# anulum/scpn-fusion-core

Measured on NVIDIA B200. Metric: converged_equilibria_per_s, higher is better.
Workload: dtype f64

## Files before the change

### scpn_fusion_core_b200/csrc/gsb_picard.cu

```cuda
#include "gsb_internal.cuh"
#include "gsb_resident.cuh"

#include <algorithm>
#include <cstdlib>

constexpr int kPT = 32;
constexpr int kTW = 8;
constexpr int kRW = 4;
constexpr int kSadChunk = 4096;
constexpr int kSadChunksMax = 64;

struct PicardState {
  int *active, *status, *iter, *cur, *best, *nxt, *xsel, *seed_active;
  double *diff_best, *gs_best, *gs_last, *diff_last, *scale;
  double *axbnd;
  double *topo;
};

struct Bufs {
  double *p[3];
};

struct gsb_picard_ws {
  int cap = 0;
// ... 890 lines not shown
  s.cur[b] = 0;
  s.best[b] = best0;
  s.nxt[b] = 1;
  s.xsel[b] = -1;
  s.seed_active[b] = (on && seed && fabs(ip[b]) >= 1e-12) ? 1 : 0;
  s.diff_best[b] = 1e9;
  s.gs_best[b] = INFINITY;
  s.gs_last[b] = INFINITY;
  s.diff_last[b] = 0.0;
  s.scale[b] = 0.0;
}

__global__ void __launch_bounds__(256)
k_seed_source(size_t n, int nr, const double *__restrict__ seedJ, double seed_sum_drdz,
              const double *__restrict__ ip, const double *__restrict__ mr,
              double *__restrict__ jphi, double *__restrict__ source,
              const int *__restrict__ seed_active) {
  const int b = blockIdx.y;
  if (!seed_active[b]) return;
  const double sc = seed_sum_drdz > 0.0 ? __ddiv_rn(ip[b], seed_sum_drdz) : 1.0;
  for (size_t i = (size_t)blockIdx.x * blockDim.x + threadIdx.x; i < n; i += (size_t)gridDim.x * blockDim.x) {
    const double j = dmul(seedJ[i], sc);
    jphi[(size_t)b * n + i] = j;
    source[(size_t)b * n + i] = dmul(mr[i % nr], j);
  }
}

__global__ void __launch_bounds__(256)
k_finalize(Bufs bufs, PicardState s, size_t n, double *__restrict__ summary, int batch,
           const int *__restrict__ mask) {
  const int b = blockIdx.y;
  if (mask && !mask[b]) return;
  const int c = s.cur[b];
  if (c != 0) {
    const double *f = bufs.p[c] + (size_t)b * n;
    double *d = bufs.p[0] + (size_t)b * n;
    for (size_t i = (size_t)blockIdx.x * blockDim.x + threadIdx.x; i < n; i += (size_t)gridDim.x * blockDim.x)
      d[i] = f[i];
  }
  if (blockIdx.x == 0 && threadIdx.x == 0 && summary) {
    double *o = summary + (size_t)b * 16;
    const double *t = s.topo + (size_t)b * 8;
    o[0] = (double)s.iter[b];
    o[1] = s.status[b] == 1 ? 1.0 : 0.0;
    o[2] = s.diff_best[b];
    o[3] = s.gs_last[b];
    o[4] = s.gs_best[b];
    o[5] = (double)s.status[b];
    o[6] = s.axbnd[2 * b];
    o[7] = s.axbnd[2 * b + 1];
    o[8] = t[0];
    o[9] = t[1];
    o[10] = t[3];
    o[11] = t[4];
    o[12] = s.diff_last[b];
    o[13] = t[6];
    o[14] = s.scale[b];
    o[15] = 0.0;
  }
}

__global__ void __launch_bounds__(256)
k_bfield(const double *__restrict__ psi, int nz, int nr, GradGeom gg, const double *__restrict__ rrow,
         double *__restrict__ br, double *__restrict__ bz) {
  const int b = blockIdx.z;
  const int ir = blockIdx.x * blockDim.x + threadIdx.x;
  const int iz = blockIdx.y * blockDim.y + threadIdx.y;
  if (ir >= nr || iz >= nz) return;
  const size_t n = (size_t)nz * nr;
  double gz, gr;
  grad_point(psi + b * n, nz, nr, iz, ir, gg, gz, gr);
  const double rs = fmax(rrow[ir], 1e-6);
  const double inv = __ddiv_rn(1.0, rs);
  br[b * n + (size_t)iz * nr + ir] = dmul(-inv, gz);
  bz[b * n + (size_t)iz * nr + ir] = dmul(inv, gr);
}


struct PicardResArgs {
  double *psi;
  const double *bc;
  const double *ip;
  const double *prof_dev;
  double *jphi;
  double *summary;
  double *hist, *gs_hist;
  double *ws_psi;
  double *ws_src;
  const double *seedJ, *cf, *mr, *rrow;
  const int *rowmask;
  double seed_sum_drdz;
  int batch, max_iter, seed, saddle, need_gs, external;
  double tol, gs_tol, alpha, oma, omega;
  double dr, dz, dr2, dz2, four_drdz;
  GradGeom gg;
  ProfileDev prof;
  int scratch_off;
  int tplane_off;
  const int *order;
  const int *n_order;
};

__device__ __forceinline__ double pl(int xo, int nz, int hw, int iz, int ir) {
  return res_pool[xo + split_index(nz, hw, iz, ir)];
}

__device__ __forceinline__ void grad_planes(int xo, int nz, int nr, int hw, int iz, int ir, const GradGeom &gg,
                                            double &gz, double &gr) {
  const double c = pl(xo, nz, hw, iz, ir);
  if (iz == 0)
    gz = ddiv_y(dsub(pl(xo, nz, hw, 1, ir), c), gg.dz, gg.inv_dz);
  else if (iz == nz - 1)
    gz = ddiv_y(dsub(c, pl(xo, nz, hw, iz - 1, ir)), gg.dz, gg.inv_dz);
  else
    gz = ddiv_y(dsub(pl(xo, nz, hw, iz + 1, ir), pl(xo, nz, hw, iz - 1, ir)), gg.two_dz, gg.inv_two_dz);
  if (ir == 0)
    gr = ddiv_y(dsub(pl(xo, nz, hw, iz, 1), c), gg.dr, gg.inv_dr);
  else if (ir == nr - 1)
    gr = ddiv_y(dsub(c, pl(xo, nz, hw, iz, ir - 1)), gg.dr, gg.inv_dr);
  else
    gr = ddiv_y(dsub(pl(xo, nz, hw, iz, ir + 1), pl(xo, nz, hw, iz, ir - 1)), gg.two_dr, gg.inv_two_dr);
}

__device__ __forceinline__ double grad_mag(const GradGeom &gg, double c, double up, double down, double left,
                                           double right, bool z_lo, bool z_hi, bool r_lo, bool r_hi) {
  double gz, gr;
  if (z_lo)
    gz = ddiv_yf(dsub(up, c), gg.dz, gg.inv_dz);
  else if (z_hi)
    gz = ddiv_yf(dsub(c, down), gg.dz, gg.inv_dz);
  else
    gz = ddiv_yf(dsub(up, down), gg.two_dz, gg.inv_two_dz);
  if (r_lo)
    gr = ddiv_yf(dsub(right, c), gg.dr, gg.inv_dr);
  else if (r_hi)
    gr = ddiv_yf(dsub(c, left), gg.dr, gg.inv_dr);
  else
    gr = ddiv_yf(dsub(right, left), gg.two_dr, gg.inv_two_dr);
  return hypot_glibc(gr, gz);
}

struct JrawK {
  double psi_ax, denom, inv_denom;
  bool hmode, same_prof;
  MtanhK mkp, mkf;
};
__device__ __forceinline__ double jraw_point(const JrawK &K, double v, double r, double cfv) {
  const double pn = ddiv_yf(dsub(v, K.psi_ax), K.denom, K.inv_denom);
  double pr = 0.0, ff = 0.0;
  if (pn >= 0.0 && pn < 1.0) {
    if (K.hmode) {
      pr = mtanh_res(pn, K.mkp);
      ff = K.same_prof ? pr : mtanh_res(pn, K.mkf);
    } else {
      pr = ff = dsub(1.0, pn);
    }
  }
  return dadd(dmul(0.5, dmul(r, pr)), dmul(0.5, dmul(cfv, ff)));
}

__device__ __forceinline__ double bcast_d(double v, int slot_off) {
  __syncthreads();
  if (threadIdx.x == 0) res_pool[slot_off] = v;
  __syncthreads();
  return res_pool[slot_off];
}

__global__ void __launch_bounds__(kResThreads, 1)
k_picard_resident(const __grid_constant__ RPlan plan, const __grid_constant__ PicardResArgs a) {
  const int lev_off = res_stage(plan);
  int nz, nr, hw, xo, f_lk, f_nch, f_rpc, f_nk;
  ResK rk;
  {
    const RLevel &F = res_level(lev_off, 0);
    nz = F.nz, nr = F.nr, hw = F.hw, xo = F.x_off, f_lk = F.lk, f_nch = F.nch, f_rpc = F.rpc, f_nk = F.nk;
    rk = res_load_resk(F.g);
  }
  const double *tab_ae = plan.lev[0].g.a_e;
  const double *tab_rs = plan.lev[0].g.r_safe, *tab_irs = plan.lev[0].g.inv_r_safe;
  const double a_ns0 = plan.lev[0].g.a_ns, a_c0 = plan.lev[0].g.a_c, inv_a_c0 = plan.lev[0].g.inv_a_c;
  const int n = nz * nr, ps = nz * hw, planes = 2 * ps, nslot = ps;
  const int tid = threadIdx.x, T = blockDim.x;
  const int lane = tid & 31, warp = tid >> 5, nw = T >> 5;
  const int step_z = T / hw, step_k = T - step_z * hw;
  const int iz_first = tid / hw, k_first = tid - iz_first * hw;
  double *sh = res_pool + a.scratch_off;
  int *shi = reinterpret_cast<int *>(sh + 32);
  const int bslot = a.scratch_off + 48;
  double *wpsi = a.ws_psi + (size_t)blockIdx.x * 3 * planes;
  double *wsrc = a.ws_src + (size_t)blockIdx.x * planes;
  const double n_all = (double)n, n_int = (double)(nz - 2) * (double)(nr - 2);
  const bool odd_nr = (nr & 1) != 0;

#define GSB_SLOT_LOOP_BEGIN()                                                  \
  for (int e = tid, iz = iz_first, k = k_first; e < nslot; e += T) {          \
    const int par_ = iz & 1;                                                   \
    const int pa = par_ * ps + e, pb = (1 - par_) * ps + e;                    \
    const bool has_odd = odd_nr ? (k < hw - 1) : true;
#define GSB_SLOT_LOOP_END()                                                    \
    k += step_k;                                                               \
    iz += step_z;                                                              \
    if (k >= hw) {                                                             \
      k -= hw;                                                                 \
      ++iz;                                                                    \
    }                                                                          \
  }

  const int n_work = a.order ? min(*a.n_order, a.batch) : a.batch;
  for (int wi = blockIdx.x; wi < n_work; wi += gridDim.x) {
    const int b = a.order ? a.order[wi] : wi;
    const double *bc = a.bc + (size_t)b * n;
    const double ipb = a.ip[b];
    double pp[4], pf[4];
#pragma unroll
    for (int i = 0; i < 4; ++i) {
      pp[i] = a.prof_dev ? a.prof_dev[(size_t)b * 8 + i] : a.prof.p[i];
      pf[i] = a.prof_dev ? a.prof_dev[(size_t)b * 8 + 4 + i] : a.prof.f[i];
    }
    const MtanhK mkp = mtanh_k(pp), mkf = mtanh_k(pf);
    const bool same_prof = pp[0] == pf[0] && pp[1] == pf[1] && pp[2] == pf[2] && pp[3] == pf[3];
    __syncthreads();
    res_load_dense(a.psi + (size_t)b * n, xo, nz, nr, hw);
    int cur = 0, best = 0, nxt = 1;
    const bool do_seed = a.seed && fabs(ipb) >= 1e-12;
    const double seed_sc = a.seed_sum_drdz > 0.0 ? __ddiv_rn(ipb, a.seed_sum_drdz) : 1.0;
    __syncthreads();
    if (a.seed) {
      for (int i = tid; i < planes; i += T) wpsi[2 * planes + i] = res_pool[xo + i];
      best = 2;
    }

    if (do_seed) {
      const double sc = seed_sc;
      for (int iz = warp; iz < nz; iz += nw)
        for (int ir = lane; ir < nr; ir += 32) {
          const double j = dmul(a.seedJ[iz * nr + ir], sc);
          wsrc[split_index(nz, hw, iz, ir)] = dmul(a.mr[ir], j);
        }
      __syncthreads();
      int p0 = xo, p1 = xo + ps, pt = a.tplane_off;
      for (int step = 0; step < 50; ++step) {
#pragma unroll 1
        for (int c = 0; c < 2; ++c) {
          const int src_plane = c == 0 ? p0 : p1;
          const int oth_plane = c == 0 ? p1 : p0;
          const int dst_plane = c == 0 ? pt : p1;
          int o = tid, iz = iz_first, k = k_first;
          while (o < nslot) {
            int vo[4], vz[4], vk[4];
            double vf[4];
#pragma unroll
            for (int u = 0; u < 4; ++u) {
              vo[u] = o, vz[u] = iz, vk[u] = k;
              const int s = (c + iz) & 1;
              const int ir = 2 * k + s;
              const bool interior = o < nslot && ir < nr && iz > 0 && iz < nz - 1 && ir > 0 && ir < nr - 1;
              vf[u] = interior ? __ldcg(wsrc + c * ps + o) : 0.0;
              o += T, k += step_k, iz += step_z;
              if (k >= hw) k -= hw, ++iz;
            }
#pragma unroll
            for (int u = 0; u < 4; ++u) {
              const int oo = vo[u], zz = vz[u];
              const int s = (c + zz) & 1;
              const int ir = 2 * vk[u] + s;
              if (oo < nslot && ir < nr) {
                double v;
                if (zz == 0 || zz == nz - 1 || ir == 0 || ir == nr - 1) {
                  v = sanitize_fast(res_pool[src_plane + oo]);
                } else {
                  const double cc = sanitize_fast(res_pool[oth_plane + oo]);
                  const double side = sanitize_fast(res_pool[oth_plane + oo - 1 + 2 * s]);
                  const double S = sanitize_fast(res_pool[oth_plane + oo - hw]), N = sanitize_fast(res_pool[oth_plane + oo + hw]);
                  const double f = sanitize_fast(vf[u]);
                  double acc = dadd(dmul(__ldg(tab_ae + ir), s ? side : cc), dmul(__ldg(tab_ae + nr + ir), s ? cc : side));
                  acc = dadd(acc, dmul(a_ns0, S));
                  acc = dadd(acc, dmul(a_ns0, N));
                  acc = dsub(acc, f);
                  v = clip_cap(ddiv_y(acc, a_c0, inv_a_c0));
                }
                res_pool[dst_plane + oo] = v;
              }
            }
          }
          __syncthreads();
        }
        const int t = p0;
        p0 = pt;
        pt = t;
      }
    }
    if (a.external && !do_seed) {
      for (int i = tid; i < planes; i += T) wsrc[i] = 0.0;
    }
    __syncthreads();
    for (int i = tid; i < planes; i += T) wpsi[(size_t)cur * planes + i] = res_pool[xo + i];
    __syncthreads();

    int status = 0, iters = 0;
    int j_slot = -1;
    bool j_ok = false;
    double diff_best = 1e9, gs_best = INFINITY, gs_last = INFINITY, diff_last = 0.0, scale = 0.0;
    double psi_ax = 0.0, psi_b = 0.0, t_izax = 0, t_irax = 0, t_izx = 0, t_irx = 0, t_found = 0;

    for (int kit = 0; kit < a.max_iter; ++kit) {
      GSB_PHASE_BEGIN();
      ValIdx mx{0.0, -1}, mb{0.0, -1};
      double mn = INFINITY;
      GSB_SLOT_LOOP_BEGIN()
        const int flat = iz * nr + 2 * k;
        const double ve = res_pool[xo + pa];
        const double vo = has_odd ? res_pool[xo + pb] : ve;
        if (ve > mx.v || mx.i < 0) mx = ValIdx{ve, flat};
        mn = fmin(mn, ve);
        if (has_odd) {
          if (vo > mx.v) mx = ValIdx{vo, flat + 1};
          mn = fmin(mn, vo);
        }
        if (__ldg(a.rowmask + iz) != 0) {
          const bool z_lo = iz == 0, z_hi = iz == nz - 1;
          {
            const double up = z_hi ? 0.0 : res_pool[xo + pb + hw], down = z_lo ? 0.0 : res_pool[xo + pb - hw];
            const double left = k > 0 ? res_pool[xo + pb - 1] : 0.0;
            const double bm = grad_mag(a.gg, ve, up, down, left, vo, z_lo, z_hi, k == 0, !has_odd);
            if (isfinite(bm)) mb = better<false>(mb, ValIdx{bm, flat});
          }
          if (has_odd) {
            const bool r_hi = 2 * k + 1 == nr - 1;
            const double up = z_hi ? 0.0 : res_pool[xo + pa + hw], down = z_lo ? 0.0 : res_pool[xo + pa - hw];
            const double right = r_hi ? 0.0 : res_pool[xo + pa + 1];
            const double bm = grad_mag(a.gg, vo, up, down, ve, right, z_lo, z_hi, false, r_hi);
            if (isfinite(bm)) mb = better<false>(mb, ValIdx{bm, flat + 1});
          }
        }
      GSB_SLOT_LOOP_END()
      mx = block_arg<true>(mx, sh, shi);
      __syncthreads();
      mb = block_arg<false>(mb, sh, shi);
      __syncthreads();
      mn = -block_max(-mn, sh);
      int xi = mb.i;
      if (a.saddle) {
        double prev_v = -1.0, best_v = INFINITY;
        int prev_i = -1, best_i = -1;
        for (int round = 0; round < 16; ++round) {
          ValIdx c{0.0, -1};
          for (int iz = warp; iz < nz; iz += nw) {
            if (!a.rowmask[iz]) continue;
            for (int ir = lane; ir < nr; ir += 32) {
              const int flat = iz * nr + ir;
              double gz, gr;
              grad_planes(xo, nz, nr, hw, iz, ir, a.gg, gz, gr);
              const double bm = hypot_glibc(gr, gz);
              if (!isfinite(bm)) continue;
              if (bm < prev_v || (bm == prev_v && flat <= prev_i)) continue;
              c = better<false>(c, ValIdx{bm, flat});
            }
          }
          __syncthreads();
          c = block_arg<false>(c, sh, shi);
          if (threadIdx.x == 0) {
            res_pool[bslot] = c.v;
            res_pool[bslot + 1] = (double)c.i;
          }
          __syncthreads();
          prev_v = res_pool[bslot];
          prev_i = (int)res_pool[bslot + 1];
          __syncthreads();
          if (prev_i < 0) break;
          const int iz = prev_i / nr, ir = prev_i - iz * nr;
          if (iz > 0 && iz < nz - 1 && ir > 0 && ir < nr - 1) {
            const double q0 = pl(xo, nz, hw, iz, ir), c2 = dmul(2.0, q0);
            const double d2r = __ddiv_rn(dadd(dsub(pl(xo, nz, hw, iz, ir + 1), c2), pl(xo, nz, hw, iz, ir - 1)), a.dr2);
            const double d2z = __ddiv_rn(dadd(dsub(pl(xo, nz, hw, iz + 1, ir), c2), pl(xo, nz, hw, iz - 1, ir)), a.dz2);
            const double drz = __ddiv_rn(dadd(dsub(dsub(pl(xo, nz, hw, iz + 1, ir + 1), pl(xo, nz, hw, iz + 1, ir - 1)),
                                                   pl(xo, nz, hw, iz - 1, ir + 1)),
                                              pl(xo, nz, hw, iz - 1, ir - 1)),
                                         a.four_drdz);
            const double det = dsub(dmul(d2r, d2z), dmul(drz, drz));
            if (isfinite(det) && det < 0.0 && prev_v < best_v) {
              best_v = prev_v;
              best_i = prev_i;
            }
          }
        }
        if (best_i >= 0) xi = best_i;
      }
      if (threadIdx.x == 0) {
        double pax = mx.v;
        if (fabs(pax) < 1e-6) pax = 1e-6;
        double px;
        double fx = 0.0, izx = 0.0, irx = 0.0;
        if (xi >= 0) {
          const int iz = xi / nr, ir = xi - iz * nr;
          px = pl(xo, nz, hw, iz, ir);
          fx = 1.0;
          izx = iz;
          irx = ir;
        } else {
          px = mn;
        }
        double pb = px;
        if (fabs(dsub(pax, pb)) < 0.1) pb = dmul(pax, 0.1);
        res_pool[bslot] = pax;
        res_pool[bslot + 1] = pb;
        res_pool[bslot + 2] = (double)(mx.i / nr);
        res_pool[bslot + 3] = (double)(mx.i % nr);
        res_pool[bslot + 4] = izx;
        res_pool[bslot + 5] = irx;
        res_pool[bslot + 6] = fx;
      }
      __syncthreads();
      psi_ax = res_pool[bslot];
      psi_b = res_pool[bslot + 1];
      t_izax = res_pool[bslot + 2];
      t_irax = res_pool[bslot + 3];
      t_izx = res_pool[bslot + 4];
      t_irx = res_pool[bslot + 5];
      t_found = res_pool[bslot + 6];
      __syncthreads();
      GSB_PHASE(48);

      if (!a.external) {
      double denom = dsub(psi_b, psi_ax);
      if (fabs(denom) < 1e-9) denom = 1e-9;
      const double inv_denom = __ddiv_rn(1.0, denom);
      const bool hmode = a.prof.hmode != 0;
      j_slot = cur;
      double acc = 0.0;
      GSB_SLOT_LOOP_BEGIN()
        const double pn_e = ddiv_yf(dsub(res_pool[xo + pa], psi_ax), denom, inv_denom);
        const double pn_o = has_odd ? ddiv_yf(dsub(res_pool[xo + pb], psi_ax), denom, inv_denom) : -1.0;
        const bool in_e = pn_e >= 0.0 && pn_e < 1.0, in_o = pn_o >= 0.0 && pn_o < 1.0;
        double pr_e = 0.0, ff_e = 0.0, pr_o = 0.0, ff_o = 0.0;
        if (in_e || in_o) {
          if (hmode) {
            const double te = mtanh_res(pn_e, mkp), to = mtanh_res(pn_o, mkp);
            double fe = te, fo = to;
            if (!same_prof) {
              fe = mtanh_res(pn_e, mkf);
              fo = mtanh_res(pn_o, mkf);
            }
            pr_e = in_e ? te : 0.0, ff_e = in_e ? fe : 0.0;
            pr_o = in_o ? to : 0.0, ff_o = in_o ? fo : 0.0;
          } else {
            pr_e = ff_e = in_e ? dsub(1.0, pn_e) : 0.0;
            pr_o = ff_o = in_o ? dsub(1.0, pn_o) : 0.0;
          }
        }
        const double je = dadd(dmul(0.5, dmul(__ldg(a.rrow + 2 * k), pr_e)), dmul(0.5, dmul(__ldg(a.cf + 2 * k), ff_e)));
        __stcg(wsrc + pa, je);
        acc += je;
        if (has_odd) {
          const double jo = dadd(dmul(0.5, dmul(__ldg(a.rrow + 2 * k + 1), pr_o)), dmul(0.5, dmul(__ldg(a.cf + 2 * k + 1), ff_o)));
          __stcg(wsrc + pb, jo);
          acc += jo;
        }
      GSB_SLOT_LOOP_END()
      acc = block_sum(acc, sh);
      const double jsum = bcast_d(acc, bslot + 8);
      const double icur = dmul(dmul(jsum, a.dr), a.dz);
      const bool ok = fabs(icur) > 1e-9;
      scale = ok ? __ddiv_rn(ipb, icur) : 0.0;
      j_ok = ok;
      {
        int e = tid, iz = iz_first, k = k_first;
        while (e < nslot) {
          double vje[4], vjo[4];
          int vpa[4], vpb[4], vk[4];
          bool vok[4], vho[4];
#pragma unroll
          for (int u = 0; u < 4; ++u) {
            const int par_ = iz & 1;
            vok[u] = e < nslot;
            vpa[u] = par_ * ps + e, vpb[u] = (1 - par_) * ps + e, vk[u] = k;
            vho[u] = odd_nr ? (k < hw - 1) : true;
            vje[u] = vok[u] ? __ldcg(wsrc + vpa[u]) : 0.0;
            vjo[u] = (vok[u] && vho[u]) ? __ldcg(wsrc + vpb[u]) : 0.0;
            e += T, k += step_k, iz += step_z;
            if (k >= hw) k -= hw, ++iz;
          }
#pragma unroll
          for (int u = 0; u < 4; ++u) {
            if (vok[u]) {
              const double je = ok ? dmul(vje[u], scale) : 0.0;
              __stcg(wsrc + vpa[u], dmul(__ldg(a.mr + 2 * vk[u]), je));
              if (vho[u]) {
                const double jo = ok ? dmul(vjo[u], scale) : 0.0;
                __stcg(wsrc + vpb[u], dmul(__ldg(a.mr + 2 * vk[u] + 1), jo));
              }
            }
          }
        }
      }
      }
      __syncthreads();
      GSB_PHASE(49);

      res_vcycle(lev_off, plan.nlev, wsrc, a.omega, 3, 3);
      __syncthreads();
      GSB_PHASE(50);

      const double *old = wpsi + (size_t)cur * planes;
      double *out = wpsi + (size_t)nxt * planes;
      double dsum = 0.0;
      int bad = 0;
      {
        int e = tid, iz = iz_first, k = k_first;
        while (e < nslot) {
          double voe[4], voo[4];
          int vpa[4], vpb[4], vk[4], vz[4];
          bool vok[4], vho[4];
#pragma unroll
          for (int u = 0; u < 4; ++u) {
            const int par_ = iz & 1;
            vok[u] = e < nslot;
            vpa[u] = par_ * ps + e, vpb[u] = (1 - par_) * ps + e, vk[u] = k, vz[u] = iz;
            vho[u] = odd_nr ? (k < hw - 1) : true;
            voe[u] = vok[u] ? __ldcg(old + vpa[u]) : 0.0;
            voo[u] = (vok[u] && vho[u]) ? __ldcg(old + vpb[u]) : 0.0;
            e += T, k += step_k, iz += step_z;
            if (k >= hw) k -= hw, ++iz;
          }
#pragma unroll
          for (int u = 0; u < 4; ++u) {
            if (vok[u]) {
              const bool zwall = vz[u] == 0 || vz[u] == nz - 1;
              {
                const bool wall = zwall || vk[u] == 0 || !vho[u];
                const double wn = wall ? bc[vz[u] * nr + 2 * vk[u]] : res_pool[xo + vpa[u]];
                const double ov = voe[u];
                if (!(fabs(wn) <= 1.79769313486231570815e308)) bad = 1;
                dsum += fabs(dsub(wn, ov));
                const double c = dadd(dmul(a.oma, ov), dmul(a.alpha, wn));
                res_pool[xo + vpa[u]] = c;
                __stcg(out + vpa[u], c);
              }
              if (vho[u]) {
                const bool wall = zwall || (2 * vk[u] + 1 == nr - 1);
                const double wn = wall ? bc[vz[u] * nr + 2 * vk[u] + 1] : res_pool[xo + vpb[u]];
                const double ov = voo[u];
                if (!(fabs(wn) <= 1.79769313486231570815e308)) bad = 1;
                dsum += fabs(dsub(wn, ov));
                const double c = dadd(dmul(a.oma, ov), dmul(a.alpha, wn));
                res_pool[xo + vpb[u]] = c;
                __stcg(out + vpb[u], c);
              }
            }
          }
        }
      }
      const int anybad = __syncthreads_or(bad);
      GSB_PHASE(51);
      double rmax = 0.0, rsq = 0.0;
      {
        const int k = tid & ((1 << f_lk) - 1), ch = tid >> f_lk;
        const int z0 = 1 + ch * f_rpc;
        const int z1 = min(z0 + f_rpc, nz - 1);
        if (ch < f_nch && k < f_nk && z0 < z1) {
          const int ce = 2 * k, co = 2 * k + 1;
          const bool e_in = ce >= 1 && ce <= nr - 2, o_in = co <= nr - 2;
          const double rs_e = __ldg(tab_rs + ce), irs_e = __ldg(tab_irs + ce);
          const double rs_o = o_in ? __ldg(tab_rs + co) : 1.0, irs_o = o_in ? __ldg(tab_irs + co) : 1.0;
          int e = z0 * hw + k;
          int par = z0 & 1;
          double ev_m = res_pool[xo + (1 - par) * ps + e - hw], od_m = res_pool[xo + par * ps + e - hw];
          double ev_0 = res_pool[xo + par * ps + e], od_0 = res_pool[xo + (1 - par) * ps + e];
          for (int iz = z0; iz < z1; ++iz) {
            const int pa = par * ps + e, pb = (1 - par) * ps + e;
            const double ev_p = res_pool[xo + pb + hw], od_p = res_pool[xo + pa + hw];
            if (e_in) {
              const double w = res_pool[xo + pb - 1];
              const double r = dsub(res_lx(rk, rs_e, irs_e, ev_0, od_0, w, ev_m, ev_p), __ldcg(wsrc + pa));
              rmax = fmax(rmax, fabs(r));
              rsq += r * r;
            }
            if (o_in) {
              const double ee = res_pool[xo + pa + 1];
              const double r = dsub(res_lx(rk, rs_o, irs_o, od_0, ee, ev_0, od_m, od_p), __ldcg(wsrc + pb));
              rmax = fmax(rmax, fabs(r));
              rsq += r * r;
            }
            ev_m = ev_0, ev_0 = ev_p;
            od_m = od_0, od_0 = od_p;
            e += hw;
            par ^= 1;
          }
        }
      }
      dsum = block_sum(dsum, sh);
      __syncthreads();
      rmax = block_max(rmax, sh);
      __syncthreads();
      rsq = block_sum(rsq, sh);
      if (threadIdx.x == 0) {
        double code = 0.0;
        double dbest = diff_best, gbest = gs_best, dl = diff_last, gl = gs_last;
        double improved = 0.0;
        if (anybad) {
          code = 3.0;
        } else {
          const double diff = dsum / n_all;
          const double gs = (rmax > 0.0 && n_int > 0.0) ? sqrt(rsq / n_int) : 0.0;
          if (a.hist) a.hist[(size_t)b * a.max_iter + kit] = diff;
          if (a.gs_hist) a.gs_hist[(size_t)b * a.max_iter + kit] = gs;
          dl = diff;
          gl = gs;
          if (gs < gbest) gbest = gs;
          if (diff < dbest) {
            dbest = diff;
            improved = 1.0;
          }
          if (diff < a.tol && (!a.need_gs || gs < a.gs_tol))
            code = 1.0;
          else if (kit + 1 >= a.max_iter)
            code = 2.0;
        }
        res_pool[bslot] = code;
        res_pool[bslot + 1] = dbest;
        res_pool[bslot + 2] = gbest;
        res_pool[bslot + 3] = dl;
        res_pool[bslot + 4] = gl;
        res_pool[bslot + 5] = improved;
      }
      __syncthreads();
      const int code = (int)res_pool[bslot];
      diff_best = res_pool[bslot + 1];
      gs_best = res_pool[bslot + 2];
      diff_last = res_pool[bslot + 3];
      gs_last = res_pool[bslot + 4];
      const bool improved = res_pool[bslot + 5] != 0.0;
      __syncthreads();
      iters = kit + 1;
      GSB_PHASE(52);
      if (blockIdx.x == 0 && threadIdx.x == 0) GSB_PHASE_COUNT(53);
      if (code == 3) {
        status = 3;
        cur = best;
        break;
      }
      const int newcur = nxt;
      if (improved) best = newcur;
      cur = newcur;
      nxt = (cur == best) ? (cur == 0 ? 1 : 0) : 3 - cur - best;
      if (code != 0) {
        status = code;
        break;
      }
    }

    {
      const double *fin = wpsi + (size_t)cur * planes;
      const double *jsrc = wpsi + (size_t)(j_slot >= 0 ? j_slot : 0) * planes;
      JrawK jk;
      jk.psi_ax = psi_ax;
      jk.denom = dsub(psi_b, psi_ax);
      if (fabs(jk.denom) < 1e-9) jk.denom = 1e-9;
      jk.inv_denom = __ddiv_rn(1.0, jk.denom);
      jk.hmode = a.prof.hmode != 0, jk.same_prof = same_prof, jk.mkp = mkp, jk.mkf = mkf;
      double *po = a.psi + (size_t)b * n;
      double *jo = a.jphi + (size_t)b * n;
      for (int iz = warp; iz < nz; iz += nw)
        for (int ir = lane; ir < nr; ir += 32) {
          const int o = split_index(nz, hw, iz, ir);
          po[iz * nr + ir] = fin[o];
          double j;
          if (j_slot >= 0)
            j = j_ok ? dmul(jraw_point(jk, __ldcg(jsrc + o), __ldg(a.rrow + ir), __ldg(a.cf + ir)), scale) : 0.0;
          else
            j = do_seed ? dmul(a.seedJ[iz * nr + ir], seed_sc) : 0.0;
          jo[iz * nr + ir] = j;
        }
      if (threadIdx.x == 0 && a.summary) {
        double *o = a.summary + (size_t)b * 16;
        o[0] = (double)iters;
        o[1] = status == 1 ? 1.0 : 0.0;
        o[2] = diff_best;
        o[3] = gs_last;
        o[4] = gs_best;
        o[5] = (double)status;
        o[6] = psi_ax;
        o[7] = psi_b;
        o[8] = t_izax;
        o[9] = t_irax;
        o[10] = t_izx;
        o[11] = t_irx;
        o[12] = diff_last;
        o[13] = t_found;
        o[14] = scale;
        o[15] = 0.0;
      }
    }
    __syncthreads();
  }
#undef GSB_SLOT_LOOP_BEGIN
#undef GSB_SLOT_LOOP_END
}

__global__ void k_fb_init(int *__restrict__ mask, int *__restrict__ order, int *__restrict__ n_order,
                          double *__restrict__ fbsum, int batch) {
  const int b = blockIdx.x * blockDim.x + threadIdx.x;
  if (b == 0) *n_order = batch;
  if (b >= batch) return;
  mask[b] = 1;
  order[b] = b;
  fbsum[4 * b] = 0.0;
  fbsum[4 * b + 1] = INFINITY;
  fbsum[4 * b + 2] = 0.0;
  fbsum[4 * b + 3] = 0.0;
}

__device__ __forceinline__ int wall_index(int nz, int nr, int iz, int ir) {
  if (iz == 0) return ir;
  if (iz == nz - 1) return nr + 2 * (nz - 2) + ir;
  return nr + 2 * (iz - 1) + (ir ? 1 : 0);
}

__global__ void __launch_bounds__(256)
k_fb_prepare(double *__restrict__ psi, const double *__restrict__ ext, const double *__restrict__ wall,
             double *__restrict__ old, size_t n, int nz, int nr, int nwall, const int *__restrict__ mask) {
  const int b = blockIdx.y;
  if (!mask[b]) return;
  double *f = psi + (size_t)b * n;
  const double *e = ext + (size_t)b * n;
  double *o = old + (size_t)b * n;
  for (size_t i = (size_t)blockIdx.x * blockDim.x + threadIdx.x; i < n; i += (size_t)gridDim.x * blockDim.x) {
    const int iz = (int)(i / nr), ir = (int)(i - (size_t)iz * nr);
    double v = f[i];
    if (iz == 0 || ir == 0 || iz == nz - 1 || ir == nr - 1) {
      v = e[i];
      if (wall) v = dadd(v, wall[(size_t)b * nwall + wall_index(nz, nr, iz, ir)]);
      f[i] = v;
    }
    o[i] = v;
  }
}

__global__ void __launch_bounds__(256)
k_fb_diff(const double *__restrict__ psi, const double *__restrict__ old, size_t n, double *__restrict__ part,
          const int *__restrict__ mask) {
  __shared__ double sh[32];
  const int b = blockIdx.y, P = gridDim.x, p = blockIdx.x;
  if (!mask[b]) return;
  const size_t i0 = n * p / P, i1 = n * (p + 1) / P;
  const double *f = psi + (size_t)b * n, *o = old + (size_t)b * n;
  double m = 0.0;
  int bad = 0;
  for (size_t i = i0 + threadIdx.x; i < i1; i += blockDim.x) {
    const double d = fabs(dsub(f[i], o[i]));
    if (d != d) bad = 1;
    m = fmax(m, d);
  }
  const int anybad = __syncthreads_or(bad);
  m = block_max(m, sh);
  if (threadIdx.x == 0) {
    part[((size_t)b * kPT + p) * 2] = m;
    part[((size_t)b * kPT + p) * 2 + 1] = anybad ? 1.0 : 0.0;
  }
}

__global__ void __launch_bounds__(1024)
k_fb_decide(const double *__restrict__ part, int P, double tol, int outer, const double *__restrict__ summary,
            double *__restrict__ fbsum, int *__restrict__ mask, int *__restrict__ order, int *__restrict__ n_order,
            int batch) {
  __shared__ int wsum[32];
  __shared__ int base;
  const int tid = threadIdx.x, lane = tid & 31, warp = tid >> 5;
  if (tid == 0) base = 0;
  __syncthreads();
  for (int b0 = 0; b0 < batch; b0 += blockDim.x) {
    const int b = b0 + tid;
    int keep = 0;
    if (b < batch && mask[b]) {
      double m = 0.0;
      bool bad = false;
      for (int q = 0; q < P; ++q) {
        m = fmax(m, part[((size_t)b * kPT + q) * 2]);
        bad = bad || part[((size_t)b * kPT + q) * 2 + 1] != 0.0;
      }
      const double diff = bad ? NAN : m;
      fbsum[4 * b] = (double)(outer + 1);
      fbsum[4 * b + 1] = diff;
      fbsum[4 * b + 2] += summary[(size_t)b * 16];
      const bool conv = diff < tol;
      fbsum[4 * b + 3] = conv ? 1.0 : 0.0;
      keep = conv ? 0 : 1;
      mask[b] = keep;
    }
    const unsigned bal = __ballot_sync(0xffffffffu, keep);
    const int pos_in_warp = __popc(bal & ((1u << lane) - 1));
    if (lane == 0) wsum[warp] = __popc(bal);
    __syncthreads();
    int off = base;
    for (int w = 0; w < warp; ++w) off += wsum[w];
    if (keep) order[off + pos_in_warp] = b;
    __syncthreads();
    if (tid == 0) {
      int t = 0;
      for (int w = 0; w < (int)(blockDim.x >> 5); ++w) t += wsum[w];
      base += t;
    }
    __syncthreads();
  }
  if (tid == 0) *n_order = base;
}

constexpr int kShapeMaxCoils = 32;
constexpr int kShapeMaxPoints = 1024;
constexpr int kShapeWarps = 4;

__global__ void __launch_bounds__(1024)
k_shape_factor(const double *__restrict__ mmat, int n, int P, double sqrt_alpha, double *__restrict__ a,
               double *__restrict__ q, double *__restrict__ rmat, double *__restrict__ q1, int *__restrict__ deficient) {
  __shared__ double sh[32];
  __shared__ double diag[kShapeMaxCoils], beta[kShapeMaxCoils];
  const int m = P + n, tid = threadIdx.x, lane = tid & 31, warp = tid >> 5, nwarps = blockDim.x >> 5;
  for (int idx = tid; idx < m * n; idx += blockDim.x) {
    const int j = idx / m, i = idx - j * m;
    a[idx] = i < P ? mmat[(size_t)j * P + i] : (i - P == j ? sqrt_alpha : 0.0);
    q[idx] = i == j ? 1.0 : 0.0;
  }
  __syncthreads();
  for (int k = 0; k < n; ++k) {
    double *col = a + (size_t)k * m;
    double s = 0.0;
    for (int i = k + tid; i < m; i += blockDim.x) s += col[i] * col[i];
    s = block_sum(s, sh);
    if (tid == 0) {
      const double sigma = sqrt(s), x0 = col[k];
      const double al = x0 >= 0.0 ? -sigma : sigma;
      diag[k] = al;
      beta[k] = sigma > 0.0 ? 1.0 / (sigma * (sigma + fabs(x0))) : 0.0;
      col[k] = x0 - al;
    }
    __syncthreads();
    for (int j = k + 1 + warp; j < n; j += nwarps) {
      double *cj = a + (size_t)j * m;
      double d = 0.0;
      for (int i = k + lane; i < m; i += 32) d += col[i] * cj[i];
      const double f = beta[k] * warp_sum(d);
      for (int i = k + lane; i < m; i += 32) cj[i] -= f * col[i];
    }
    __syncthreads();
  }
  for (int k = n - 1; k >= 0; --k) {
    const double *col = a + (size_t)k * m;
    for (int j = warp; j < n; j += nwarps) {
      double *cj = q + (size_t)j * m;
      double d = 0.0;
      for (int i = k + lane; i < m; i += 32) d += col[i] * cj[i];
      const double f = beta[k] * warp_sum(d);
      for (int i = k + lane; i < m; i += 32) cj[i] -= f * col[i];
    }
    __syncthreads();
  }
  for (int idx = tid; idx < P * n; idx += blockDim.x) {
    const int p = idx / n, j = idx - p * n;
    q1[idx] = q[(size_t)j * m + p];
  }
  for (int idx = tid; idx < n * n; idx += blockDim.x) {
    const int i = idx / n, j = idx - i * n;
    rmat[idx] = i == j ? diag[i] : (i < j ? a[(size_t)j * m + i] : 0.0);
  }
  if (tid == 0) {
    double mx = 0.0;
    bool bad = false;
    for (int i = 0; i < n; ++i) {
      bad = bad || !isfinite(diag[i]);
      mx = fmax(mx, fabs(diag[i]));
    }
    for (int i = 0; i < n; ++i) bad = bad || !(fabs(diag[i]) > (double)n * 2.220446049250313e-16 * mx);
    *deficient = bad ? 1 : 0;
  }
}

__device__ __forceinline__ double np_pairwise_leaf(const double *a, int n) {
  if (n < 8) {
    double r = 0.0;
    for (int i = 0; i < n; ++i) r = dadd(r, a[i]);
    return r;
  }
  double r[8];
#pragma unroll
  for (int j = 0; j < 8; ++j) r[j] = a[j];
  int i = 8;
  for (; i < n - (n % 8); i += 8)
#pragma unroll
    for (int j = 0; j < 8; ++j) r[j] = dadd(r[j], a[i + j]);
  double res = dadd(dadd(dadd(r[0], r[1]), dadd(r[2], r[3])), dadd(dadd(r[4], r[5]), dadd(r[6], r[7])));
  for (; i < n; ++i) res = dadd(res, a[i]);
  return res;
}
template <int D>
__device__ __forceinline__ double np_pairwise_dev(const double *a, int n) {
  if constexpr (D == 0) {
    return np_pairwise_leaf(a, n);
  } else {
    if (n <= 128) return np_pairwise_leaf(a, n);
    int n2 = n / 2;
    n2 -= n2 % 8;
    return dadd(np_pairwise_dev<D - 1>(a, n2), np_pairwise_dev<D - 1>(a + n2, n - n2));
  }
}

__device__ __forceinline__ double warp_min_d(double v) {
#pragma unroll
  for (int o = 16; o > 0; o >>= 1) v = fmin(v, __shfl_xor_sync(0xffffffffu, v, o));
  return v;
}

__global__ void __launch_bounds__(256)
k_shape_target(const double *__restrict__ psi, size_t n, int nr, const double *__restrict__ wts,
               const int *__restrict__ corner, int P, const double *__restrict__ explicit_t, double *__restrict__ out,
               const int *__restrict__ mask) {
  __shared__ double smp[kShapeMaxPoints];
  __shared__ double mean;
  const int b = blockIdx.x;
  if (!mask[b]) return;
  double *o = out + (size_t)b * (2 * P + 4);
  if (explicit_t) {
    for (int p = threadIdx.x; p < P; p += blockDim.x) o[p] = explicit_t[(size_t)b * P + p];
    return;
  }
  const double *f = psi + (size_t)b * n;
  for (int p = threadIdx.x; p < P; p += blockDim.x) {
    const double *c = f + corner[p];
    const double *w = wts + 4 * p;
    smp[p] = dadd(dadd(dadd(dmul(w[0], c[0]), dmul(w[1], c[1])), dmul(w[2], c[nr])), dmul(w[3], c[nr + 1]));
  }
  __syncthreads();
  if (threadIdx.x == 0) mean = __ddiv_rn(np_pairwise_dev<4>(smp, P), (double)P);
  __syncthreads();
  for (int p = threadIdx.x; p < P; p += blockDim.x) o[p] = mean;
}
// ... 1137 lines not shown
```

Baseline: 4139.

## Carry next iteration's max and gradient argmin from the residual pass

Computes the next iteration's psi maximum (interior plus wall points) and boundary-gradient argmin at the end of each Picard iteration, so the separate scan at the start of the next iteration can be skipped. The dsum/rmax/rsq and two argmax/argmin reductions are merged into a single warp-shuffle plus shared-memory pass with one barrier, in place of several sequential block reductions. If NaNs are present the carried values are discarded and the full scan runs again. The minimum still needs a light rescan when no gradient candidate exists. This adds register pressure and extra shared-memory slots, and tie-breaking across the merged reductions has to match the old behaviour.

```diff
diff --git a/scpn_fusion_core_b200/csrc/gsb_picard.cu b/scpn_fusion_core_b200/csrc/gsb_picard.cu
--- a/scpn_fusion_core_b200/csrc/gsb_picard.cu
+++ b/scpn_fusion_core_b200/csrc/gsb_picard.cu
@@ -1216,11 +1216,14 @@
     bool j_ok = false;
     double diff_best = 1e9, gs_best = INFINITY, gs_last = INFINITY, diff_last = 0.0, scale = 0.0;
     double psi_ax = 0.0, psi_b = 0.0, t_izax = 0, t_irax = 0, t_izx = 0, t_irx = 0, t_found = 0;
+    ValIdx mx{0.0, -1}, mb{0.0, -1};
+    bool carried = false, carried_no_mb = false;
 
     for (int kit = 0; kit < a.max_iter; ++kit) {
       GSB_PHASE_BEGIN();
-      ValIdx mx{0.0, -1}, mb{0.0, -1};
       double mn = INFINITY;
+      if (!carried) {
+      mx = ValIdx{0.0, -1}, mb = ValIdx{0.0, -1};
       GSB_SLOT_LOOP_BEGIN()
         const int flat = iz * nr + 2 * k;
         const double ve = res_pool[xo + pa];
@@ -1253,6 +1256,13 @@
       mb = block_arg<false>(mb, sh, shi);
       __syncthreads();
       mn = -block_max(-mn, sh);
+      } else if (carried_no_mb) {
+        GSB_SLOT_LOOP_BEGIN()
+          mn = fmin(mn, res_pool[xo + pa]);
+          if (has_odd) mn = fmin(mn, res_pool[xo + pb]);
+        GSB_SLOT_LOOP_END()
+        mn = -block_max(-mn, sh);
+      }
       int xi = mb.i;
       if (a.saddle) {
         double prev_v = -1.0, best_v = INFINITY;
@@ -1467,6 +1477,8 @@
       const int anybad = __syncthreads_or(bad);
       GSB_PHASE(51);
       double rmax = 0.0, rsq = 0.0;
+      ValIdx tx{0.0, -1}, tb{0.0, -1};
+      int psi_nan = 0;
       {
         const int k = tid & ((1 << f_lk) - 1), ch = tid >> f_lk;
         const int z0 = 1 + ch * f_rpc;
@@ -1478,6 +1490,7 @@
           const double rs_o = o_in ? __ldg(tab_rs + co) : 1.0, irs_o = o_in ? __ldg(tab_irs + co) : 1.0;
           int e = z0 * hw + k;
           int par = z0 & 1;
+          int flat = z0 * nr + ce;
           double ev_m = res_pool[xo + (1 - par) * ps + e - hw], od_m = res_pool[xo + par * ps + e - hw];
           double ev_0 = res_pool[xo + par * ps + e], od_0 = res_pool[xo + (1 - par) * ps + e];
           for (int iz = z0; iz < z1; ++iz) {
@@ -1495,18 +1508,74 @@
               rmax = fmax(rmax, fabs(r));
               rsq += r * r;
             }
+            psi_nan |= isnan(ev_0) | isnan(od_0);
+            tx = better<true>(tx, ValIdx{ev_0, flat});
+            tx = better<true>(tx, ValIdx{od_0, flat + 1});
             ev_m = ev_0, ev_0 = ev_p;
             od_m = od_0, od_0 = od_p;
             e += hw;
+            flat += nr;
             par ^= 1;
           }
         }
-      }
-      dsum = block_sum(dsum, sh);
-      __syncthreads();
-      rmax = block_max(rmax, sh);
-      __syncthreads();
-      rsq = block_sum(rsq, sh);
+        const int n_wall = 2 * nr + (odd_nr ? nz - 2 : 0);
+        for (int j = tid; j < n_wall; j += T) {
+          const bool zrow = j < 2 * nr;
+          const int iz = zrow ? (j < nr ? 0 : nz - 1) : j - 2 * nr + 1;
+          const int ir = zrow ? (j < nr ? j : j - nr) : nr - 1;
+          const int fl = iz * nr + ir;
+          const double v = pl(xo, nz, hw, iz, ir);
+          psi_nan |= isnan(v);
+          tx = better<true>(tx, ValIdx{v, fl});
+        }
+      }
+      GSB_SLOT_LOOP_BEGIN()
+        if (__ldg(a.rowmask + iz) != 0) {
+          const int flat = iz * nr + 2 * k;
+          const double ve = res_pool[xo + pa];
+          const double vo = has_odd ? res_pool[xo + pb] : ve;
+          const bool z_lo = iz == 0, z_hi = iz == nz - 1;
+          {
+            const double up = z_hi ? 0.0 : res_pool[xo + pb + hw], down = z_lo ? 0.0 : res_pool[xo + pb - hw];
+            const double left = k > 0 ? res_pool[xo + pb - 1] : 0.0;
+            const double bm = grad_mag(a.gg, ve, up, down, left, vo, z_lo, z_hi, k == 0, !has_odd);
+            if (isfinite(bm)) tb = better<false>(tb, ValIdx{bm, flat});
+          }
+          if (has_odd) {
+            const bool r_hi = 2 * k + 1 == nr - 1;
+            const double up = z_hi ? 0.0 : res_pool[xo + pa + hw], down = z_lo ? 0.0 : res_pool[xo + pa - hw];
+            const double right = r_hi ? 0.0 : res_pool[xo + pa + 1];
+            const double bm = grad_mag(a.gg, vo, up, down, ve, right, z_lo, z_hi, false, r_hi);
+            if (isfinite(bm)) tb = better<false>(tb, ValIdx{bm, flat + 1});
+          }
+        }
+      GSB_SLOT_LOOP_END()
+      static_assert(kResThreads / 32 <= 16, "the combined reduction keeps 16 partials per member");
+      dsum = warp_sum(dsum);
+      rmax = warp_max(rmax);
+      rsq = warp_sum(rsq);
+      tx = warp_arg<true>(tx);
+      tb = warp_arg<false>(tb);
+      int *shx = reinterpret_cast<int *>(sh + 80);
+      if (lane == 0) {
+        sh[warp] = dsum;
+        sh[16 + warp] = rmax;
+        sh[32 + warp] = rsq;
+        sh[48 + warp] = tx.v;
+        sh[64 + warp] = tb.v;
+        shx[warp] = tx.i;
+        shx[16 + warp] = tb.i;
+      }
+      const bool next_nan = __syncthreads_or(psi_nan) != 0;
+      if (warp == 0) {
+        dsum = warp_sum(lane < nw ? sh[lane] : 0.0);
+        rmax = warp_max(lane < nw ? sh[16 + lane] : -INFINITY);
+        rsq = warp_sum(lane < nw ? sh[32 + lane] : 0.0);
+        tx = warp_arg<true>(lane < nw ? ValIdx{sh[48 + lane], shx[lane]} : ValIdx{0.0, -1});
+        tb = warp_arg<false>(lane < nw ? ValIdx{sh[64 + lane], shx[16 + lane]} : ValIdx{0.0, -1});
+      }
+      mx = tx;
+      mb = tb;
       if (threadIdx.x == 0) {
         double code = 0.0;
         double dbest = diff_best, gbest = gs_best, dl = diff_last, gl = gs_last;
@@ -1536,6 +1605,7 @@
         res_pool[bslot + 3] = dl;
         res_pool[bslot + 4] = gl;
         res_pool[bslot + 5] = improved;
+        res_pool[bslot + 6] = tb.i < 0 ? 1.0 : 0.0;
       }
       __syncthreads();
       const int code = (int)res_pool[bslot];
@@ -1544,6 +1614,8 @@
       diff_last = res_pool[bslot + 3];
       gs_last = res_pool[bslot + 4];
       const bool improved = res_pool[bslot + 5] != 0.0;
+      carried = !next_nan;
+      carried_no_mb = res_pool[bslot + 6] != 0.0;
       __syncthreads();
       iters = kit + 1;
       GSB_PHASE(52);
```

After: 4122 (median of 6 runs). No clear change (-0.4%).
